# xinge008/SCDA

Measured on AMD Instinct MI355X. Metric: images/sec (fwd+bwd) VGG16 Faster-RCNN+SCDA 512x1024, higher is better.
Workload: dtype f32; 1 GPU; vgg16_FasterRCNN + 4-cluster SCDA, synthetic Cityscapes->Foggy 512x1024, batch=1/GPU (BASELINE.json configs[1]); 1 step = 1 source + 1 target image, 4 optimiser phases; gt_boxes=12, rois=512, clusters=4, recon=256, parallelism=dp1

## Files before the change

include/scda_ops.h:

```cpp
#ifndef SCDA_OPS_H
#define SCDA_OPS_H

#include <stddef.h>
#include <stdint.h>

#ifdef __cplusplus
extern "C" {
#endif

#define SCDA_OK 0
#define SCDA_EINVAL (-1)
#define SCDA_ELAUNCH (-2)
#define SCDA_ENODEV (-3)

int scda_version(void);
int scda_device_count(void);
const char *scda_last_error(void);

void scda_prof_enable(unsigned kernel_mask);
int scda_prof_num_kernels(void);
const char *scda_prof_kernel_name(int k);
int scda_prof_collect(long long *launches, double *ms, double *flops, double *bytes);
void scda_debug_last_plan(int *out4);
void scda_debug_plan_conv(int dir, int batch, int Cin, int IH, int IW, int Cout, int KH, int KW, int S, int P, int row_period,
// ... 46 lines not shown
int scda_bbox_overlaps_hip(const float *boxes, int N, const float *query, int K, float *out, void *stream);

int scda_anchor_label_hip(const float *anchors, int KA, const float *gts, int G, int gt_stride, float neg_thresh, float pos_thresh,
                          float min_gt_best, float *best_iou, int *best_gt, unsigned *gt_best, signed char *labels, int *pos_list,
                          int *neg_list, int *counts, void *stream);
int scda_anchor_finalize_hip(signed char *labels, const int *best_gt, const int *pos_list, const int *drop_pos, int n_drop_pos,
                             const int *neg_list, const int *drop_neg, int n_drop_neg, const double *anchors64, const float *gts,
                             int gt_stride, int A, int fh, int fw, long long *cls_targets, float *loc_targets, float *loc_masks,
                             void *stream);
int scda_proposal_decode_hip(const int *order, const float *exp_wh, int n, const double *anchors64, const float *loc, const float *prob, int A, int fh,
                             int fw, double img_h, double img_w, double min_size, float *props5, unsigned char *ok, void *stream);
int scda_proposal_gather_hip(const float *props5, const long long *keep, const long long *num_keep, float image_index, int max_rows,
                             float *out6, void *stream);
int scda_proposal_match_hip(const float *props, int n_prop, int prop_stride, const float *gts, int G, int gt_stride, float img_h,
                            float img_w, float pos_thresh, float neg_hi, float neg_lo, float *rois, float *best_iou, int *best_gt,
                            signed char *labels, int *pos_list, int *neg_list, int *counts, void *stream);
int scda_proposal_finalize_hip(const float *cand_rois, const int *sel, const int *gt_of, const float *enc, const float *gts,
                               int gt_stride, int R, int num_classes, float image_index, float *rois5, long long *labels,
                               float *loc_targets, float *loc_weights, void *stream);

int scda_kmeans_capacity(void);
int scda_kmeans_hip(const float *rois, int roi_stride, int N, int k, int first_index, const double *uniforms_host, int trials,
                    float *centres, int *labels, int *counts, int *members, int *seed_index, int *n_iter, int *status, void *stream);
int scda_cluster_gather_hip(const float *feats, long long feat_stride, int N, int F, const int *members, const int *counts,
                            const int *picks_or_null, int k, int threshold, float *out, void *stream);

size_t scda_rpn_topk_workspace_bytes(int B, int KA, int top_n);
int scda_rpn_topk_hip(const float *prob, int B, int A, int fh, int fw, int top_n, int *order, void *ws, void *stream);
int scda_rpn_decode_batched_hip(const int *order, int n, const double *anchors64, const float *loc, const float *prob, int B, int A,
                                int fh, int fw, const float *image_info, int info_stride, double min_size, float *props5,
                                unsigned char *ok, void *stream);
size_t scda_rpn_proposals_workspace_bytes(int B, int A, int fh, int fw, int top_n);
int scda_rpn_proposals_hip(const float *prob, const float *loc, const double *anchors64, int B, int A, int fh, int fw,
                           const float *image_info, int info_stride, int pre_nms_top_n, double min_size, float nms_thresh,
                           int post_nms_top_n, void *ws, float *rois5, float *props6, int *counts, void *stream);
size_t scda_box_predict_workspace_bytes(int B, int P, int C);
int scda_box_predict_hip(const float *rois, const int *roi_counts, int B, int P, const float *prob, const float *loc, int C,
                         const float *image_info, int info_stride, const double *stds_host, const double *means_host,
                         float score_thresh, float nms_thresh, int top_n, void *ws, float *det, int *det_counts, void *stream);
int scda_soft_nms_capacity(void);
int scda_soft_nms_segments_hip(float *boxes, const long long *seg, int S, int max_n, int method, float sigma, float Nt, float threshold,
                               int64_t *keep, int64_t *num_out, void *stream);
int scda_box_predict_soft_hip(const float *rois, const int *roi_counts, int B, int P, const float *prob, const float *loc, int C,
                              const float *image_info, int info_stride, const double *stds_host, const double *means_host,
                              float score_thresh, int top_n, int method, float sigma, float Nt, float threshold, void *ws, float *det,
                              int *det_counts, void *stream);

int scda_det_rois_hip(const float *detections, const int *detection_counts, int B, int top_n, float *rois5, int *cls, void *stream);
int scda_mask_select_hip(const float *logits, long long stride_r, long long stride_c, long long stride_h, long long stride_w,
                         const int *cls, int R, int C, int ph, int pw, int sigmoid, float *out, void *stream);
int scda_mask_paste_hip(const float *rois, int roi_stride, const int *cls_or_null, const float *planes, int R, int ph, int pw, int H,
                        int W, int packed, float threshold, void *out, void *stream);
int scda_mask_rescale_max_ratio(void);
int scda_mask_rescale_hip(const float *rois, int roi_stride, const int *cls_or_null, const float *planes, int R, int ph, int pw, int H,
                          int W, const float *image_info, int info_stride, int masks_per_image, int Ho, int Wo, int packed,
                          float threshold, void *out, float *foot_rois, int *status, void *stream);

size_t scda_keypoint_decode_workspace_bytes(int R, int Kp, int W);
int scda_keypoint_decode_hip(const float *rois, int roi_stride, const int *cls_or_null, const float *heat, long long stride_r,
                             long long stride_k, long long stride_h, long long stride_w, int R, int Kp, int ph, int pw, int H, int W,
                             void *workspace, float *out, void *stream);

int scda_keypoint_ce_fwd_hip(const float *heat, long long stride_r, long long stride_k, int R, int Kp, int HW, const int *targets,
                             float *stats, float *row_loss, float *out2, void *stream);
int scda_keypoint_ce_bwd_hip(const float *heat, long long stride_r, long long stride_k, int R, int Kp, int HW, const int *targets,
                             const float *stats, const float *out2, const float *grad_scalar, float *dheat, long long dstride_r,
                             long long dstride_k, void *stream);

int scda_mask_rle_max_chars(int h, int w);
size_t scda_mask_rle_workspace_bytes(int R, int H, int Wd, int cap_runs);
int scda_mask_rle_hip(const uint32_t *bits, int R, int H, int Wd, const float *image_info, int info_stride, int masks_per_image,
                      int h_all, int w_all, const float *rois_or_null, int roi_stride, int cap_runs, int cap_bytes, void *ws,
                      int *n_runs, uint32_t *counts, int *n_bytes, unsigned char *chars, uint32_t *area, uint32_t *bbox, void *stream);
size_t scda_mask_iou_workspace_bytes(int M, int N, int H, int Wd);
int scda_mask_iou_hip(const uint32_t *dt_bits, int M, const uint32_t *gt_bits, int N, int H, int Wd, int h, int w,
                      const unsigned char *iscrowd_or_null, void *ws, double *iou, uint32_t *inter, void *stream);

size_t scda_mask_frpoly_workspace_bytes(int P, int Q, int H, int Wd);
int scda_mask_frpoly_hip(const double *xy, int V, const int *poly_first, const int *poly_plane, int P, const uint32_t *rle_counts, int C,
                         const int *rle_first, const int *rle_plane, int Q, const int *sizes, int N, int H, int Wd, void *ws,
                         uint32_t *bits, uint32_t *area_or_null, void *stream);

int scda_coco_det_rows_hip(const float *detections, const int *detection_counts, int B, int top_n, const uint32_t *mask_area_or_null,
                           int K, double *dt_xywh, double *dt_area, float *score, int *cat, void *stream);
int scda_coco_box_iou_hip(const double *dt, const int *dt_counts, const double *gt, const int *gt_counts, const unsigned char *iscrowd,
                          int B, int D, int G, double *iou, void *stream);
int scda_coco_match_hip(const double *iou, int B, int D, int G, const int *dt_counts, const int *dt_cat, const float *score,
                        const double *dt_area, const int *gt_counts, const int *gt_cat, const double *gt_area,
                        const unsigned char *gt_iscrowd, int K, const double *iou_thrs, int T, const double *area_rng, int A, int max_det,
                        int *rank, uint32_t *bits, int *npig, int *seen, int *dbg_match_or_null, void *stream);
int scda_coco_match_ign_hip(const double *iou, int B, int D, int G, const int *dt_counts, const int *dt_cat, const float *score,
                            const double *dt_area, const int *gt_counts, const int *gt_cat, const double *gt_area,
                            const unsigned char *gt_iscrowd, const unsigned char *gt_ignore_or_null, int K, const double *iou_thrs, int T,
                            const double *area_rng, int A, int max_det, int *rank, uint32_t *bits, int *npig, int *seen,
                            int *dbg_match_or_null, void *stream);
int scda_coco_kp_rows_hip(const float *detections, const int *detection_counts, int B, int top_n, const float *keypoints, int Kp, int K,
                          double *dt_xywh, double *dt_area, float *score, int *cat, void *stream);
int scda_coco_oks_hip(const float *dt_keypoints, const int *dt_counts, const double *gt_keypoints, const double *gt_boxes,
                      const double *gt_areas, const int *gt_counts, const double *vars, int Kp, const unsigned char *gt_iscrowd_or_null,
                      const int *gt_num_keypoints_or_null, int B, int D, int G, double *oks, unsigned char *gt_ignore_or_null,
                      void *stream);
int scda_coco_prop_rows_hip(const float *proposals, const int *proposal_counts, int B, int P, int xyxy_as_xywh, double *dt_xywh,
                            double *dt_area, float *score, int *cat, void *stream);
int scda_coco_regroup_hip(int B, int D, int G, int K, const int *dt_counts, const double *in_xywh, const double *in_area,
                          const float *in_score, const int *in_cat, const int *gt_counts, const int *gt_cat, const double *gt_area,
                          const unsigned char *gt_iscrowd, const double *in_iou, double *dt_xywh, double *dt_area, float *score, int *cat,
                          double *out_gt_area, unsigned char *out_gt_iscrowd, int *out_gt_cat, double *out_iou, int *perm_dets,
                          int *perm_gts, void *stream);
size_t scda_coco_accumulate_workspace_bytes(int n_images, int D, int K, int A);
int scda_coco_accumulate_hip(const int *image_ids, int n_images, int D, const int *cat, const int *rank, const float *score,
                             const uint32_t *bits, const int *npig, const int *seen, int K, int T, int A, const double *rec_thrs, int R,
                             const int *max_dets, int M, int max_det_last, void *ws, double *precision, double *recall, double *scores,
                             void *stream);
int scda_coco_summarize_hip(const double *precision, const double *recall, int T, int R, int K, int A, int M, const int *spec,
                            int n_stats, double *stats, void *stream);

int scda_map_rows_hip(const float *detections, const int *detection_counts, int B, int D, const float *image_info, int info_w,
                      int scale_column, int num_classes, int keep_num, int *box, float *score, int *cls, int *rank, int *kept, int *tp,
                      int *dbg_match_or_null, int G, int *dbg_claimed_or_null, void *stream);
int scda_map_match_hip(const int *box, const int *cls, const int *rank, const int *kept, int B, int D, const int *gt_boxes,
                       const int *gt_counts, int G, int num_classes, double iou_thr, int *tp, int *gt_num, int *dbg_match_or_null,
                       int *dbg_claimed_or_null, void *stream);
int scda_map_recall_hip(const float *proposals, const int *proposal_counts, int B, int P, int prop_w, const float *gts,
                        const int *gt_counts, int Gr, int gt_w, int *counters, void *stream);
size_t scda_map_accumulate_workspace_bytes(int n_images, int D);
int scda_map_accumulate_hip(int n_images, int D, const float *score, const int *cls, const int *rank, const int *kept, const int *tp,
                            const int *sum_gt, int num_classes, void *ws, double *ap, double *max_recall, int *rows, void *stream);

int scda_eval_place_rows_hip(const void *src, int W, int cap, int row_words, const int *order_host, const int *counts_host_or_null,
                             const int *counts_dev_or_null, int start, int max_images, int fill, void *dst, int *flags, void *stream);
int scda_eval_sum_counters_hip(const int *src, int W, int n, int *dst, void *stream);
size_t scda_eval_mark_duplicates_workspace_bytes(int n);
int scda_eval_mark_duplicates_hip(const int *image_ids, int n, void *ws, int *first, int *flags, int raise_on_duplicate, void *stream);
int scda_map_merge_duplicates_hip(const int *first, int n, int D, const int *box, const float *score, const int *cls, const int *rank,
                                  const int *kept, int *tp, int *flags, void *stream);

size_t scda_conv2d_workspace_bytes(int batch, int Cin, int IH, int IW, int Cout, int KH, int KW, int S, int P);
size_t scda_conv2d_packed_elems(int Cout, int Cin, int KH, int KW, int for_dgrad);
int scda_conv2d_pack_weight_hip(const float *w, float *out, int Cout, int Cin, int KH, int KW, int for_dgrad,
                                void *stream);
long long scda_conv2d_pack_tiles(int Cout, int Cin, int KH, int KW, int for_dgrad);
int scda_conv2d_pack_weights_batched_hip(const float *base, float *out, const long long *desc, int n, long long n_tiles,
                                         void *stream);
int scda_conv2d_fwd_hip(const float *x, const float *wp, const float *bias , float *y, int batch,
                        int Cin, int IH, int IW, int Cout, int KH, int KW, int S, int P, int row_period, int act, float slope,
                        void *ws, size_t ws_bytes, void *stream);
int scda_conv2d_dgrad_hip(const float *dy, const float *wt, float *dx, int batch, int Cin, int IH, int IW, int Cout,
                          int KH, int KW, int S, int P, int row_period, void *ws, size_t ws_bytes, void *stream);
int scda_conv2d_dgrad_act_hip(const float *dy, const float *wt, float *dx, int batch, int Cin, int IH, int IW, int Cout,
                              int KH, int KW, int S, int P, int row_period, const float *act_src, float act_slope, void *ws,
                              size_t ws_bytes, void *stream);
int scda_conv2d_dgrad_small_cin_hip(const float *dy, const float *w, float *dx, int batch, int Cin, int IH, int IW, int Cout,
                                    int KH, int KW, int S, int P, void *stream);
int scda_conv2d_wgrad_hip(const float *dy, const float *x, float *dw, int batch, int Cin, int IH, int IW, int Cout,
                          int KH, int KW, int S, int P, int row_period, int accumulate, void *ws, size_t ws_bytes, void *stream);
int scda_conv2d_wgrad_bias_fusable(int batch, int Cout, int OH, int OW, const float *dy);
int scda_conv2d_wgrad_bias_hip(const float *dy, const float *x, float *dw, float *db, int batch, int Cin, int IH, int IW,
                               int Cout, int KH, int KW, int S, int P, int row_period, int accumulate, int db_accumulate, void *ws,
                               size_t ws_bytes, void *stream);

int scda_conv2d_wino_supported(int batch, int C, int H, int W, int M);
size_t scda_conv2d_wino_packed_elems(int Cout, int Cin, int for_dgrad);
int scda_conv2d_wino_pack_hip(const float *w, float *out, int Cout, int Cin, int for_dgrad, void *stream);
int scda_conv2d_wino_hip(const float *x, const float *u, const float *bias, float *y, int batch, int C, int H, int W, int M, int act,
                         float slope, const float *mask_src, float mask_slope, int for_dgrad, void *ws, size_t ws_bytes, void *stream);

int scda_conv2d_wino_stacked_hip(const float *x, const float *u, const float *bias, float *y, int maps, int C, int M, int act, float slope,
                                 const float *mask_src, float mask_slope, int for_dgrad, void *ws, size_t ws_bytes, void *stream);
int scda_conv2d_wino_pool_hip(const float *x, const float *u, const float *bias, float *pool_y, unsigned char *pool_idx, int batch, int C,
                              int H, int W, int M, int act, float slope, void *stream);
int scda_conv2d_wino_wgrad_supported(int batch, int Cin, int H, int W, int Cout);
int scda_conv2d_wino_wgrad_hip(const float *dy, const float *x, float *dw, float *db, int batch, int Cin, int H, int W, int Cout,
                               int accumulate, int db_accumulate, void *ws, size_t ws_bytes, void *stream);
int scda_conv2d_wino_wgrad_stacked_hip(const float *dy, const float *x, float *dw, float *db, int maps, int Cin, int Cout, int accumulate,
                                       int db_accumulate, void *ws, size_t ws_bytes, void *stream);

size_t scda_gemm_workspace_bytes(int M, int N, int K);
int scda_gemm_hip(const float *A, const float *B, float *C, int M, int N, int K, int lda, int ldb, int ldc,
                  int trans_a, int trans_b, const float *bias, int bias_on_n, int act, float slope, int accumulate,
                  void *ws, size_t ws_bytes, void *stream);

int scda_maxpool2x2_fwd_hip(const float *x, float *y, uint8_t *idx, int planes, int H, int W, void *stream);
int scda_maxpool2x2_bwd_hip(const float *dy, const uint8_t *idx, float *dx, int planes, int H, int W, void *stream);
int scda_maxpool3x3s2_fwd_hip(const float *x, float *y, int planes, int H, int W, void *stream);
int scda_add_relu_hip(const float *a, const float *b, float *y, long long n, void *stream);
int scda_maxpool2x2_bwd_relu_hip(const float *dy, const uint8_t *idx, const float *y_pooled, float *dx, int planes, int H, int W,
                                 void *stream);
int scda_act_fwd_hip(const float *x, float *y, long long n, int mode, float slope, void *stream);
int scda_act_bwd_hip(const float *dy, const float *y, float *dx, long long n, int mode, float slope, void *stream);
int scda_axpby_hip(const float *a, const float *b, float *y, long long n, float alpha, float beta, void *stream);
int scda_dropout_mask_hip(uint8_t *mask, long long n, float p, uint64_t seed, void *stream);
int scda_dropout_apply_hip(const float *x, const uint8_t *mask, float *y, long long n, float scale, void *stream);
int scda_dropout_seeded_hip(const float *x, float *y, long long n, float p, uint64_t seed, float scale, const float *relu_src,
                            void *stream);
int scda_sigmoid_bce_rows_fwd_hip(const float *x, const float *t, int t_rows, const float *w, int C, int n, float scale,
                                  int accumulate, float *prob_out, float *out1, void *stream);
int scda_sigmoid_bce_rows_bwd_hip(const float *prob, const float *t, int t_rows, const float *w, int C, int n, float scale,
                                  const float *grad_scalar, float *dx, void *stream);
size_t scda_bias_grad_workspace_bytes(int C);
int scda_bias_grad_nchw_hip(const float *dy, float *db, int B, int C, int HW, int accumulate, float *ws, void *stream);
int scda_colsum_hip(const float *dy, float *db, int M, int N, int accumulate, void *stream);
int scda_softmax_ce_fwd_hip(const float *logits, const int64_t *targets, int R, int C, int ignore_index, float *probs,
                            float *out2, void *stream);
int scda_softmax_ce_bwd_hip(const float *probs, const int64_t *targets, int R, int C, int ignore_index,
                            const float *fwd_out2, const float *grad_scalar, float *dlogits, void *stream);
int scda_row_softmax_hip(const float *x, float *y, int R, int C, void *stream);
int scda_accuracy_hip(const float *logits, const int64_t *targets, int R, int C, int ignore_index, float *out1,
                      void *stream);
size_t scda_smooth_l1_workspace_bytes(void);
int scda_smooth_l1_fwd_hip(const float *pred, const float *mask, const float *target, long long n, float sigma,
                           float scale, float *partial_ws, float *out1, void *stream);
int scda_smooth_l1_bwd_hip(const float *pred, const float *mask, const float *target, long long n, float sigma,
                           float scale, const float *grad_scalar, float *dpred, void *stream);
int scda_instnorm_fwd_hip(const float *x, float *y, float *mean, float *rstd, int planes, int HW, float eps, int act,
                          float slope, void *stream);
int scda_instnorm_bwd_hip(const float *dy, const float *x, const float *mean, const float *rstd, float *dx, int planes,
                          int HW, int act, float slope, void *stream);
int scda_instnorm_drop_add_fwd_hip(const float *x, const float *residual, float *y, float *mean, float *rstd, int planes, int HW,
                                   float eps, float p, uint64_t seed, float scale , void *stream);
int scda_instnorm_drop_bwd_hip(const float *dy, const float *x, const float *mean, const float *rstd, float *dx, int planes, int HW,
                               float p, uint64_t seed, float scale, void *stream);
int scda_instnorm_drop_add_fwd_dev_hip(const float *x, const float *residual, float *y, float *mean, float *rstd, int planes, int HW,
                                       float eps, float p, const uint64_t *seed_dev, float scale, void *stream);
int scda_instnorm_drop_bwd_dev_hip(const float *dy, const float *x, const float *mean, const float *rstd, float *dx, int planes, int HW,
                                   float p, const uint64_t *seed_dev, float scale, void *stream);
size_t scda_batchnorm_workspace_bytes(int B, int C, int HW);
int scda_batchnorm_fwd_hip(const float *x, float *y, const float *gamma, const float *beta, float *running_mean,
                           float *running_var, float *save_mean, float *save_rstd, int B, int C, int HW, float eps,
                           float momentum, int act, float slope, float *ws, void *stream);
int scda_batchnorm_bwd_hip(const float *dy, const float *x, const float *gamma, const float *beta, const float *save_mean,
                           const float *save_rstd, float *dx, float *dgamma, float *dbeta, int B, int C, int HW, int act,
                           float slope, int accumulate, float *ws, void *stream);
int scda_batchnorm_add_relu_ok(int B, int HW);
int scda_batchnorm_add_relu_fwd_hip(const float *x, const float *residual, float *y, const float *gamma, const float *beta,
                                    float *running_mean, float *running_var, float *save_mean, float *save_rstd, int B, int C,
                                    int HW, float eps, float momentum, void *stream);
int scda_batchnorm_add_relu_bwd_hip(const float *dy, const float *x, const float *y, const float *gamma, const float *beta,
                                    const float *save_mean, const float *save_rstd, float *dx_or_null, float *d_residual,
                                    float *dgamma, float *dbeta, int B, int C, int HW, int accumulate, void *stream);
int scda_batchnorm_eval_hip(const float *x, const float *dy_or_null, float *out, const float *gamma, const float *beta,
                            const float *running_mean, const float *running_var, int B, int C, int HW, float eps, int act,
                            float slope, void *stream);
int scda_upsample2x_fwd_hip(const float *x, float *y, int planes, int IH, int IW, void *stream);
int scda_upsample2x_bwd_hip(const float *dy, float *dx, int planes, int IH, int IW, void *stream);
int scda_instnorm_up2_supported(int IH, int IW);
int scda_instnorm_up2_fwd_hip(const float *x, float *y2, float *mean, float *rstd, int planes, int IH, int IW, float eps, int act,
                              float slope, void *stream);
int scda_instnorm_drop_add_up2_fwd_hip(const float *x, const float *residual, float *y2, float *mean, float *rstd, int planes, int IH,
                                       int IW, float eps, float p, uint64_t seed, float scale , void *stream);
int scda_instnorm_drop_add_up2_fwd_dev_hip(const float *x, const float *residual, float *y2, float *mean, float *rstd, int planes,
                                           int IH, int IW, float eps, float p, const uint64_t *seed_dev, float scale, void *stream);
int scda_instnorm_up2_bwd_hip(const float *dy2, const float *x, const float *mean, const float *rstd, float *dx, int planes, int IH,
                              int IW, int act, float slope, void *stream);
int scda_instnorm_drop_up2_bwd_hip(const float *dy2, const float *x, const float *mean, const float *rstd, float *dx, float *dresidual,
                                   int planes, int IH, int IW, float p, uint64_t seed, float scale, void *stream);
int scda_instnorm_drop_up2_bwd_dev_hip(const float *dy2, const float *x, const float *mean, const float *rstd, float *dx,
                                       float *dresidual, int planes, int IH, int IW, float p, const uint64_t *seed_dev, float scale,
                                       void *stream);
int scda_bce_fwd_hip(const float *p, const float *t, int n, float *out1, void *stream);
int scda_bce_bwd_hip(const float *p, const float *t, int n, const float *grad_scalar, float *dp, void *stream);
int scda_avg2x2s1_fwd_hip(const float *x, float *y, int planes, int H, int W, void *stream);
int scda_avg2x2s1_bwd_hip(const float *dy, float *dx, int planes, int H, int W, void *stream);
int scda_gap_fwd_hip(const float *x, float *y, int planes, int HW, void *stream);
int scda_gap_bwd_hip(const float *dy, float *dx, int planes, int HW, void *stream);
int scda_row_mean_hip(const float *x, float *y, int R, int C, void *stream);
int scda_adam_hip(float *param, const float *grad, float *exp_avg, float *exp_avg_sq, long long n, float lr,
                  float beta1, float beta2, float eps, float weight_decay, int step, void *stream);
int scda_adam_limited_hip(float *param, const float *grad, float *exp_avg, float *exp_avg_sq, long long n, float lr,
                          float beta1, float beta2, float eps, float weight_decay, int step, int max_blocks, void *stream);

size_t scda_image_resize_tmp_bytes(int rows, int out_w, int C);
int scda_image_resize_normalize_hip(const unsigned char *src, int H, int W, int C, const int *bounds_h, const int *kk_h,
                                    int ksize_h, int out_w, const int *bounds_v, const int *kk_v, int ksize_v, int out_h,
                                    int row0, int rows, unsigned char *tmp, size_t tmp_bytes, int normalize, float mean,
                                    float stdv, int flip, float *out, void *stream);

#ifdef __cplusplus
}
#endif
#endif
```

scda_amd/native.py:

```python
import ctypes
import os
import re
import weakref

import torch

_HERE = os.path.dirname(os.path.abspath(__file__))
LIB_PATH = os.environ.get("SCDA_OPS_LIB") or os.path.join(_HERE, "libscda_ops.so")
HEADER_PATH = os.path.join(os.path.dirname(_HERE), "include", "scda_ops.h")

_lib = None


class ScdaNativeError(RuntimeError):
    pass


C_SCALARS = {"int": ctypes.c_int, "unsigned": ctypes.c_uint, "float": ctypes.c_float, "double": ctypes.c_double,
             "long long": ctypes.c_longlong, "size_t": ctypes.c_size_t, "uint64_t": ctypes.c_uint64}
C_RETURNS = dict(C_SCALARS, **{"void": None, "const char *": ctypes.c_char_p})


def parse_header(text):
    text = re.sub(r"/\*.*?\*/", " ", text, flags=re.S)
# ... 1088 lines not shown
    return bool(lib().scda_conv2d_wino_enabled())


def _route(direction, B, Cin, IH, IW, Cout, KH, KW, stride, pad, row_period):
    pool, maps = ctypes.c_int(0), ctypes.c_int(0)
    fam = lib().scda_conv2d_route(direction, B, Cin, IH, IW, Cout, KH, KW, stride, pad, row_period, ctypes.byref(pool), ctypes.byref(maps))
    return fam, bool(pool.value), maps.value


def wino_stacked(B, IH, IW, row_period):
    return _route(0, B, 0, IH, IW, 0, 3, 3, 1, 1, row_period)[2]


def wino_ok(B, Cin, IH, IW, Cout, KH, KW, stride, pad, row_period=0):
    return _route(0, B, Cin, IH, IW, Cout, KH, KW, stride, pad, row_period)[0] != 0


def wino_wgrad_ok(B, Cin, IH, IW, Cout, KH, KW, stride, pad, row_period=0):
    return _route(2, B, Cin, IH, IW, Cout, KH, KW, stride, pad, row_period)[0] != 0


def conv2d_wino_wgrad(dy, x, w_shape, out=None, db_out=None, want_bias=False, row_period=0):
    _req(dy, "dy"); _req(x, "x")
    B, Cin, IH, IW = x.shape
    Cout = w_shape[0]
    acc = dbacc = 0
    if out is None:
        out = torch.empty(tuple(w_shape), dtype=torch.float32, device=x.device)
    else:
        _req(out, "out"); acc = 1
    db = None
    if want_bias or db_out is not None:
        if db_out is None:
            db = torch.empty(Cout, dtype=torch.float32, device=x.device)
        else:
            _req(db_out, "db_out"); db = db_out; dbacc = 1
    ws, n = _conv_ws(B, Cin, IH, IW, Cout, 3, 3, 1, 1, x.device)
    if row_period:
        maps = wino_stacked(B, IH, IW, row_period)
        if not maps:
            raise ValueError("conv2d_wino_wgrad: row_period %d on %s is not a stack of 7 x 7 maps" % (row_period, tuple(x.shape)))
        _check(lib().scda_conv2d_wino_wgrad_stacked_hip(_p(dy), _p(x), _p(out), _p(db), maps, Cin, Cout, acc, dbacc, _p(ws), n, _stream()),
               "scda_conv2d_wino_wgrad_stacked_hip")
        return out, db
    _check(lib().scda_conv2d_wino_wgrad_hip(_p(dy), _p(x), _p(out), _p(db), B, Cin, IH, IW, Cout, acc, dbacc, _p(ws), n, _stream()),
           "scda_conv2d_wino_wgrad_hip")
    return out, db


def conv2d_wino_pack(w, for_dgrad=False, cache=True):
    _req(w, "w")
    Cout, Cin, KH, KW = w.shape
    cache = cache and isinstance(w, torch.nn.Parameter)
    key = (w.data_ptr(), 2 + int(for_dgrad))
    flat = getattr(w, "_scda_flat", None)
    tag = (w._version, flat.epoch if flat is not None else WEIGHT_EPOCH[0], tuple(w.shape))
    if cache:
        hit = _PACK_CACHE.get(key)
        if hit is not None and hit[0] == tag and hit[2]() is w:
            return hit[1]
    L = lib()
    n = L.scda_conv2d_wino_packed_elems(Cout, Cin, int(for_dgrad))
    out = torch.empty(n, dtype=torch.float32, device=w.device)
    _check(L.scda_conv2d_wino_pack_hip(_p(w.contiguous()), _p(out), Cout, Cin, int(for_dgrad), _stream()), "scda_conv2d_wino_pack_hip")
    if cache:
        _PACK_CACHE[key] = (tag, out, weakref.ref(w))
    return out


def conv2d_wino(x, u, bias, M, act=ACT_NONE, slope=0.01, mask_src=None, mask_slope=0.0, for_dgrad=False, row_period=0):
    B, C, H, W = x.shape
    y = torch.empty(B, M, H, W, dtype=torch.float32, device=x.device)
    ws, n = _conv_ws(B, C, H, W, M, 3, 3, 1, 1, x.device)
    if row_period:
        maps = wino_stacked(B, H, W, row_period)
        if not maps:
            raise ValueError("conv2d_wino: row_period %d on %s is not a stack of 7 x 7 maps" % (row_period, tuple(x.shape)))
        _check(lib().scda_conv2d_wino_stacked_hip(_p(x), _p(u), _p(bias), _p(y), maps, C, M, act, slope, _p(mask_src), mask_slope,
                                                  int(for_dgrad), _p(ws), n, _stream()), "scda_conv2d_wino_stacked_hip")
        return y
    _check(lib().scda_conv2d_wino_hip(_p(x), _p(u), _p(bias), _p(y), B, C, H, W, M, act, slope, _p(mask_src), mask_slope, int(for_dgrad),
                                      _p(ws), n, _stream()), "scda_conv2d_wino_hip")
    return y


def conv_pool_fusable(B, Cin, IH, IW, Cout, KH, KW, stride, pad, row_period=0):
    return _route(0, B, Cin, IH, IW, Cout, KH, KW, stride, pad, row_period)[1]


def conv2d_wino_pool(x, u, bias, M, act=ACT_NONE, slope=0.01):
    B, C, H, W = x.shape
    y = torch.empty(B, M, H // 2, W // 2, dtype=torch.float32, device=x.device)
    idx = torch.empty(B, M, H // 2, W // 2, dtype=torch.uint8, device=x.device)
    _check(lib().scda_conv2d_wino_pool_hip(_p(x), _p(u), _p(bias), _p(y), _p(idx), B, C, H, W, M, act, slope, _stream()),
           "scda_conv2d_wino_pool_hip")
    return y, idx


def conv2d_pack_all(flat):
    ws = getattr(flat, "conv_weights", None)
    if not ws:
        return
    wino = tuple(bool(getattr(w, "_scda_wino_used", False)) for w in ws) if wino_enabled() else None
    plans = flat.__dict__.setdefault("_scda_pack_plans", {})
    plan = plans.get(wino)
    L = lib()
    if plan is None:
        rows, entries, off, tiles = [], [], 0, 0
        base = flat.data.data_ptr()
        for i, w in enumerate(ws):
            Cout, Cin, KH, KW = w.shape
            src = (w.data_ptr() - base) // 4
            use_wino = wino is not None and wino[i] and all(L.scda_conv2d_packed_elems(Cout, Cin, KH, KW, d) for d in (2, 3))
            for d in ((2, 3) if use_wino else (0, 1)):
                n = int(L.scda_conv2d_packed_elems(Cout, Cin, KH, KW, d))
                rows.append([src, off, Cout, Cin, KH * KW, d, tiles])
                entries.append((w, d if d >= 2 else bool(d), off, n))
                off += n
                tiles += int(L.scda_conv2d_pack_tiles(Cout, Cin, KH, KW, d))
        desc = upload(torch.tensor(rows, dtype=torch.int64), flat.data.device)
        while len(plans) >= 4:
            plans.pop(next(iter(plans)))
        plan = (desc, off, entries, tiles, wino)
    else:
        plans.pop(wino)
    plans[wino] = plan
    desc, total, entries, tiles, _ = plan
    out = flat.__dict__.get("_scda_pack_out")
    if out is None or out.numel() < total:
        out = flat.__dict__["_scda_pack_out"] = torch.empty(total, dtype=torch.float32, device=flat.data.device)
    _check(L.scda_conv2d_pack_weights_batched_hip(_p(flat.data), _p(out), _p(desc), len(entries), tiles, _stream()),
           "scda_conv2d_pack_weights_batched_hip")
    for w, d, off, n in entries:
        if w.data_ptr() < flat.data.data_ptr():
            continue
        _PACK_CACHE[(w.data_ptr(), d)] = ((w._version, flat.epoch, tuple(w.shape)), out[off:off + n], weakref.ref(w))


def conv2d_fwd(x, w, bias, stride, pad, act=ACT_NONE, slope=0.01, row_period=0):
    _req(x, "x"); _req(w, "w")
    if bias is not None:
        _req(bias, "bias")
    B, Cin, IH, IW = x.shape
    Cout, Cin2, KH, KW = w.shape
    if Cin2 != Cin:
        raise ValueError(f"conv2d: input has {Cin} channels, weight expects {Cin2}")
    OH = (IH + 2 * pad - KH) // stride + 1
    OW = (IW + 2 * pad - KW) // stride + 1
    use_wino = wino_ok(B, Cin, IH, IW, Cout, KH, KW, stride, pad, row_period)
    if isinstance(w, torch.nn.Parameter):
        w._scda_wino_used = use_wino
    if use_wino:
        return conv2d_wino(x, conv2d_wino_pack(w, False), bias, Cout, act, slope, row_period=row_period)
    wp = conv2d_pack_weight(w, False)
    y = torch.empty(B, Cout, OH, OW, dtype=torch.float32, device=x.device)
    ws, n = _conv_ws(B, Cin, IH, IW, Cout, KH, KW, stride, pad, x.device)
    _check(lib().scda_conv2d_fwd_hip(_p(x), _p(wp), _p(bias), _p(y), B, Cin, IH, IW, Cout, KH, KW, stride, pad, row_period, act, slope,
                                     _p(ws), n, _stream()), "scda_conv2d_fwd_hip")
    return y


def conv2d_dgrad(dy, w, x_shape, stride, pad, act_src=None, act_slope=0.0, row_period=0):
    _req(dy, "dy"); _req(w, "w")
    B, Cin, IH, IW = x_shape
    Cout, _, KH, KW = w.shape
    if act_src is not None:
        _req(act_src, "act_src")
        if tuple(act_src.shape) != tuple(x_shape):
            raise ValueError("act_src must have the shape of the conv input")
    if _route(1, B, Cin, IH, IW, Cout, KH, KW, stride, pad, row_period)[0]:
        return conv2d_wino(dy, conv2d_wino_pack(w, True), None, Cin, ACT_NONE, 0.0, act_src, act_slope, for_dgrad=True, row_period=row_period)
    dx = torch.empty(B, Cin, IH, IW, dtype=torch.float32, device=dy.device)
    if act_src is None and Cin <= 4 and Cout * KH * KW * 16 <= 65536 and (KH, KW) in ((3, 3), (1, 1)):
        _check(lib().scda_conv2d_dgrad_small_cin_hip(_p(dy), _p(w.contiguous()), _p(dx), B, Cin, IH, IW, Cout, KH, KW, stride, pad,
                                                     _stream()), "scda_conv2d_dgrad_small_cin_hip")
        return dx
    wt = conv2d_pack_weight(w, True)
    ws, n = _conv_ws(B, Cin, IH, IW, Cout, KH, KW, stride, pad, dy.device)
    _check(lib().scda_conv2d_dgrad_act_hip(_p(dy), _p(wt), _p(dx), B, Cin, IH, IW, Cout, KH, KW, stride, pad, row_period, _p(act_src),
                                           act_slope, _p(ws), n, _stream()), "scda_conv2d_dgrad_act_hip")
    return dx


def conv2d_wgrad(dy, x, w_shape, stride, pad, out=None, row_period=0):
    _req(dy, "dy"); _req(x, "x")
    B, Cin, IH, IW = x.shape
    Cout, _, KH, KW = w_shape
    if wino_wgrad_ok(B, Cin, IH, IW, Cout, KH, KW, stride, pad, row_period):
        return conv2d_wino_wgrad(dy, x, w_shape, out=out, row_period=row_period)[0]
    acc = 0
    if out is None:
        out = torch.empty(tuple(w_shape), dtype=torch.float32, device=x.device)
    else:
        _req(out, "out"); acc = 1
    ws, n = _conv_ws(B, Cin, IH, IW, Cout, KH, KW, stride, pad, x.device)
    _check(lib().scda_conv2d_wgrad_hip(_p(dy), _p(x), _p(out), B, Cin, IH, IW, Cout, KH, KW, stride, pad, row_period, acc, _p(ws), n,
                                       _stream()), "scda_conv2d_wgrad_hip")
    return out


def conv2d_wgrad_bias(dy, x, w_shape, stride, pad, out=None, db_out=None, row_period=0):
    _req(dy, "dy"); _req(x, "x")
    B, Cin, IH, IW = x.shape
    Cout, _, KH, KW = w_shape
    if wino_wgrad_ok(B, Cin, IH, IW, Cout, KH, KW, stride, pad, row_period):
        return conv2d_wino_wgrad(dy, x, w_shape, out=out, db_out=db_out, want_bias=True, row_period=row_period)
    L = lib()
    if not L.scda_conv2d_wgrad_bias_fusable(B, Cout, dy.shape[2], dy.shape[3], _p(dy)):
        return conv2d_wgrad(dy, x, w_shape, stride, pad, out=out, row_period=row_period), bias_grad_nchw(dy, out=db_out)
    acc = dbacc = 0
    if out is None:
        out = torch.empty(tuple(w_shape), dtype=torch.float32, device=x.device)
    else:
        _req(out, "out"); acc = 1
    if db_out is None:
        db_out = torch.empty(Cout, dtype=torch.float32, device=x.device)
    else:
        _req(db_out, "db_out"); dbacc = 1
    ws, n = _conv_ws(B, Cin, IH, IW, Cout, KH, KW, stride, pad, x.device)
    _check(L.scda_conv2d_wgrad_bias_hip(_p(dy), _p(x), _p(out), _p(db_out), B, Cin, IH, IW, Cout, KH, KW, stride, pad, row_period, acc,
                                        dbacc, _p(ws), n, _stream()), "scda_conv2d_wgrad_bias_hip")
    return out, db_out


def gemm(a, b, M, N, K, lda, ldb, trans_a=False, trans_b=False, bias=None, bias_on_n=True, act=ACT_NONE, slope=0.01,
         out=None, accumulate=False):
    _req(a, "a"); _req(b, "b")
    if out is None:
        if accumulate:
            raise ValueError("accumulate needs out")
        out = torch.empty(M, N, dtype=torch.float32, device=a.device)
    else:
        _req(out, "out")
    L = lib()
    n = L.scda_gemm_workspace_bytes(M, N, K)
    ws = workspace(n, a.device)
    _check(L.scda_gemm_hip(_p(a), _p(b), _p(out), M, N, K, lda, ldb, N, int(trans_a), int(trans_b), _p(bias), int(bias_on_n), act, slope,
                           int(accumulate), _p(ws), n, _stream()), "scda_gemm_hip")
    return out


def linear_fwd(x, w, bias, act=ACT_NONE):
    M, K = x.shape
    N = w.shape[0]
    return gemm(x, w, M, N, K, K, K, False, False, bias, True, act)


def linear_dgrad(dy, w):
    M, K = dy.shape
    N = w.shape[1]
    return gemm(dy, w, M, N, K, K, N, False, True)


def linear_wgrad(dy, x, out=None, accumulate=True):
    Kb, M = dy.shape
    N = x.shape[1]
    return gemm(dy, x, M, N, Kb, M, N, True, True, out=out, accumulate=out is not None and accumulate)


def maxpool2x2_fwd(x):
    _req(x, "x")
    B, C, H, W = x.shape
    y = torch.empty(B, C, H // 2, W // 2, dtype=torch.float32, device=x.device)
    idx = torch.empty(B, C, H // 2, W // 2, dtype=torch.uint8, device=x.device)
    _check(lib().scda_maxpool2x2_fwd_hip(_p(x), _p(y), _p(idx), B * C, H, W, _stream()), "scda_maxpool2x2_fwd_hip")
    return y, idx


def maxpool2x2_bwd(dy, idx, x_shape, relu_y=None):
    _req(dy, "dy"); _req(idx, "idx", torch.uint8)
    B, C, H, W = x_shape
    dx = torch.empty(B, C, H, W, dtype=torch.float32, device=dy.device)
    if relu_y is None:
        _check(lib().scda_maxpool2x2_bwd_hip(_p(dy), _p(idx), _p(dx), B * C, H, W, _stream()), "scda_maxpool2x2_bwd_hip")
    else:
        _req(relu_y, "relu_y")
        _check(lib().scda_maxpool2x2_bwd_relu_hip(_p(dy), _p(idx), _p(relu_y), _p(dx), B * C, H, W, _stream()),
               "scda_maxpool2x2_bwd_relu_hip")
    return dx


def maxpool3x3s2_fwd(x):
    _req(x, "x")
    B, C, H, W = x.shape
    y = torch.empty(B, C, (H - 1) // 2 + 1, (W - 1) // 2 + 1, dtype=torch.float32, device=x.device)
    _check(lib().scda_maxpool3x3s2_fwd_hip(_p(x), _p(y), B * C, H, W, _stream()), "scda_maxpool3x3s2_fwd_hip")
    return y


def add_relu(a, b):
    _req(a, "a"); _req(b, "b")
    if a.shape != b.shape:
        raise ValueError("add_relu: shape mismatch")
    y = torch.empty_like(a)
    _check(lib().scda_add_relu_hip(_p(a), _p(b), _p(y), a.numel(), _stream()), "scda_add_relu_hip")
    return y


ACT_MODE = {"relu": 0, "leaky": 1, "tanh": 2, "sigmoid": 3}


def act_fwd(x, mode, slope=0.01):
    _req(x, "x")
    y = torch.empty_like(x)
    _check(lib().scda_act_fwd_hip(_p(x), _p(y), x.numel(), mode, slope, _stream()), "scda_act_fwd_hip")
    return y


def act_bwd(dy, y, mode, slope=0.01):
    _req(dy, "dy"); _req(y, "y")
    dx = torch.empty_like(dy)
    _check(lib().scda_act_bwd_hip(_p(dy), _p(y), _p(dx), dy.numel(), mode, slope, _stream()), "scda_act_bwd_hip")
    return dx


def axpby(a, b, alpha=1.0, beta=1.0):
    _req(a, "a")
    if b is not None:
        _req(b, "b")
    y = torch.empty_like(a)
    _check(lib().scda_axpby_hip(_p(a), _p(b), _p(y), a.numel(), alpha, beta, _stream()), "scda_axpby_hip")
    return y


def dropout_mask(shape, p, seed, device):
    mask = torch.empty(shape, dtype=torch.uint8, device=device)
    _check(lib().scda_dropout_mask_hip(_p(mask), mask.numel(), p, seed & 0xFFFFFFFFFFFFFFFF, _stream()), "scda_dropout_mask_hip")
    return mask


def dropout_apply(x, mask, scale):
    _req(x, "x"); _req(mask, "mask", torch.uint8)
    y = torch.empty_like(x)
    _check(lib().scda_dropout_apply_hip(_p(x), _p(mask), _p(y), x.numel(), scale, _stream()), "scda_dropout_apply_hip")
    return y


def dropout_seeded(x, p, seed, scale, relu_src=None):
    _req(x, "x")
    if relu_src is not None:
        _req(relu_src, "relu_src")
    y = torch.empty_like(x)
    _check(lib().scda_dropout_seeded_hip(_p(x), _p(y), x.numel(), p, seed & 0xFFFFFFFFFFFFFFFF, scale, _p(relu_src), _stream()),
           "scda_dropout_seeded_hip")
    return y


def sigmoid_bce_rows_fwd(x, t, w, scale, out=None, want_prob=True):
    _req(x, "x"); _req(t, "t")
    C, n = x.shape
    t_rows = t.numel() // n
    if t.numel() != t_rows * n or t_rows not in (1, C):
        raise ValueError("labels must be [1,n] or [C,n]")
    if w is not None:
        _req(w, "w")
    acc = out is not None
    if out is None:
        out = torch.empty(1, dtype=torch.float32, device=x.device)
    prob = torch.empty_like(x) if want_prob else None
# ... 454 lines not shown
```

Before: 113.2 images/s.

## Add dedicated thin-channel 1x1 conv kernels for fwd, dgrad and wgrad

```diff
diff --git a/include/scda_ops.h b/include/scda_ops.h
--- a/include/scda_ops.h
+++ b/include/scda_ops.h
@@ -222,6 +222,14 @@
                               size_t ws_bytes, void *stream);
 int scda_conv2d_dgrad_small_cin_hip(const float *dy, const float *w, float *dx, int batch, int Cin, int IH, int IW, int Cout,
                                     int KH, int KW, int S, int P, void *stream);
+int scda_conv1x1_thin_ok(int batch, int Cin, int IH, int IW, int Cout, int KH, int KW, int S, int P, int row_period);
+int scda_conv1x1_thin_fwd_hip(const float *x, const float *w, const float *bias , float *y, int batch, int Cin, int HW,
+                              int Cout, int act, float slope, void *stream);
+int scda_conv1x1_thin_dgrad_hip(const float *dy, const float *w, float *dx, int batch, int Cin, int HW, int Cout, const float *act_src,
+                                float act_slope, void *stream);
+size_t scda_conv1x1_thin_wgrad_workspace_bytes(int batch, int Cin, int HW, int Cout);
+int scda_conv1x1_thin_wgrad_hip(const float *dy, const float *x, float *dw, float *db, int batch, int Cin, int HW, int Cout,
+                                int accumulate, int db_accumulate, void *ws, size_t ws_bytes, void *stream);
 int scda_conv2d_wgrad_hip(const float *dy, const float *x, float *dw, int batch, int Cin, int IH, int IW, int Cout,
                           int KH, int KW, int S, int P, int row_period, int accumulate, void *ws, size_t ws_bytes, void *stream);
 int scda_conv2d_wgrad_bias_fusable(int batch, int Cout, int OH, int OW, const float *dy);
diff --git a/scda_amd/csrc/conv_thin.hip b/scda_amd/csrc/conv_thin.hip
--- /dev/null
+++ b/scda_amd/csrc/conv_thin.hip
@@ -0,0 +1,332 @@
+#include <hip/hip_runtime.h>
+#include <stdint.h>
+
+#include <algorithm>
+
+#include "common.h"
+#include "launch_plan.h"
+#include "mfma_tile.h"
+
+namespace scda {
+
+constexpr int THIN_MAX = 4;
+constexpr int THIN_LDS_ROWS = 1024;
+constexpr long long THIN_MIN_PIXELS = 65536;
+constexpr int THIN_WG_FC = 8;
+constexpr int THIN_WG_STRIP = 1024;
+
+template <int PX> struct PxVec;
+template <> struct PxVec<4> {
+    static __device__ __forceinline__ void load(const float *p, float v[4]) { const float4 t = *reinterpret_cast<const float4 *>(p); v[0] = t.x; v[1] = t.y; v[2] = t.z; v[3] = t.w; }
+    static __device__ __forceinline__ void store(float *p, const float v[4]) { *reinterpret_cast<float4 *>(p) = make_float4(v[0], v[1], v[2], v[3]); }
+};
+template <> struct PxVec<1> {
+    static __device__ __forceinline__ void load(const float *p, float v[1]) { v[0] = *p; }
+    static __device__ __forceinline__ void store(float *p, const float v[1]) { *p = v[0]; }
+};
+
+__device__ __forceinline__ void thin_stage_weights(const float *__restrict__ w, double *wl, const int rows, const int cols, const int srow,
+                                                   const int scol) {
+    for (int i = threadIdx.x; i < rows * THIN_MAX; i += blockDim.x) {
+        const int r = i >> 2, c = i & 3;
+        wl[i] = c < cols ? (double)w[(size_t)r * srow + (size_t)c * scol] : 0.0;
+    }
+    __syncthreads();
+}
+
+template <int M, int PX>
+__global__ __launch_bounds__(256) void conv1x1_thin_rows_kernel(const float *__restrict__ in, const float *__restrict__ w, const int sm,
+                                                                const int sk, const float *__restrict__ bias, float *__restrict__ out,
+                                                                const long long groups, const int K, const int HW, const int act,
+                                                                const float slope, const float *__restrict__ mask_src,
+                                                                const float mask_slope) {
+    extern __shared__ __attribute__((aligned(16))) double thin_wl[];
+    double *part = thin_wl + (size_t)K * THIN_MAX;
+    thin_stage_weights(w, thin_wl, K, M, sk, sm);
+    const int lane = threadIdx.x & 63, wave = __builtin_amdgcn_readfirstlane(threadIdx.x >> 6);
+    const int kq = (K + 3) >> 2, k0 = wave * kq, k1 = min(K, k0 + kq);
+    const int gpi = HW / PX;
+    const long long tiles = (groups + 63) >> 6;
+    for (long long tile = blockIdx.x; tile < tiles; tile += gridDim.x) {
+        const long long gidx = tile * 64 + lane;
+        const bool live = gidx < groups;
+        const long long b = live ? gidx / gpi : 0;
+        const int p = live ? (int)(gidx - b * gpi) * PX : 0;
+        const float *src = in + (size_t)b * K * HW + p;
+        double acc[M][PX];
+#pragma unroll
+        for (int m = 0; m < M; ++m)
+#pragma unroll
+            for (int j = 0; j < PX; ++j) acc[m][j] = 0.0;
+        if (live) {
+#pragma unroll 8
+            for (int k = k0; k < k1; ++k) {
+                float v[PX];
+                PxVec<PX>::load(src + (size_t)k * HW, v);
+#pragma unroll
+                for (int m = 0; m < M; ++m) {
+                    const double a = thin_wl[k * THIN_MAX + m];
+#pragma unroll
+                    for (int j = 0; j < PX; ++j) acc[m][j] = fma(a, (double)v[j], acc[m][j]);
+                }
+            }
+        }
+        if (wave > 0) {
+#pragma unroll
+            for (int m = 0; m < M; ++m)
+#pragma unroll
+                for (int j = 0; j < PX; ++j) part[((wave - 1) * (M * PX) + m * PX + j) * 64 + lane] = acc[m][j];
+        }
+        __syncthreads();
+        if (wave == 0 && live) {
+#pragma unroll
+            for (int m = 0; m < M; ++m) {
+                const size_t o = ((size_t)b * M + m) * HW + p;
+                float r[PX], ms[PX];
+                if (mask_src) PxVec<PX>::load(mask_src + o, ms);
+#pragma unroll
+                for (int j = 0; j < PX; ++j) {
+                    double t = acc[m][j];
+#pragma unroll
+                    for (int q = 0; q < 3; ++q) t += part[(q * (M * PX) + m * PX + j) * 64 + lane];
+                    float x = (float)(bias ? t + (double)bias[m] : t);
+                    x = apply_act(x, act, slope);
+                    if (mask_src) x = ms[j] > 0.f ? x : x * mask_slope;
+                    r[j] = x;
+                }
+                PxVec<PX>::store(out + o, r);
+            }
+        }
+        __syncthreads();
+    }
+}
+
+template <int K, int PX>
+__global__ __launch_bounds__(256) void conv1x1_thin_k_kernel(const float *__restrict__ in, const float *__restrict__ w, const int sm,
+                                                             const int sk, const float *__restrict__ bias, float *__restrict__ out,
+                                                             const long long groups, const int M, const int mper, const int HW,
+                                                             const int act, const float slope, const float *__restrict__ mask_src,
+                                                             const float mask_slope) {
+    extern __shared__ __attribute__((aligned(16))) double thin_wl[];
+    const int m0 = blockIdx.y * mper, m1 = min(M, m0 + mper);
+    thin_stage_weights(w + (size_t)m0 * sm, thin_wl, m1 - m0, K, sm, sk);
+    const int gpi = HW / PX;
+    for (long long gidx = blockIdx.x * 256LL + threadIdx.x; gidx < groups; gidx += gridDim.x * 256LL) {
+        const long long b = gidx / gpi;
+        const int p = (int)(gidx - b * gpi) * PX;
+        double v[K][PX];
+#pragma unroll
+        for (int k = 0; k < K; ++k) {
+            float t[PX];
+            PxVec<PX>::load(in + ((size_t)b * K + k) * HW + p, t);
+#pragma unroll
+            for (int j = 0; j < PX; ++j) v[k][j] = (double)t[j];
+        }
+#pragma unroll 4
+        for (int m = m0; m < m1; ++m) {
+            const size_t o = ((size_t)b * M + m) * HW + p;
+            float r[PX], ms[PX];
+            if (mask_src) PxVec<PX>::load(mask_src + o, ms);
+            const double bm = bias ? (double)bias[m] : 0.0;
+#pragma unroll
+            for (int j = 0; j < PX; ++j) {
+                double a = 0.0;
+#pragma unroll
+                for (int k = 0; k < K; ++k) a = fma(thin_wl[(m - m0) * THIN_MAX + k], v[k][j], a);
+                float x = (float)(bias ? a + bm : a);
+                x = apply_act(x, act, slope);
+                if (mask_src) x = ms[j] > 0.f ? x : x * mask_slope;
+                r[j] = x;
+            }
+            PxVec<PX>::store(out + o, r);
+        }
+    }
+}
+
+template <int TC, int PX>
+__global__ __launch_bounds__(256) void conv1x1_thin_wgrad_kernel(const float *__restrict__ T, const float *__restrict__ F, const int FC_all,
+                                                                 const long long npix, const int HW, double *__restrict__ part) {
+    constexpr int FC = THIN_WG_FC, NV = TC * FC + TC + FC;
+    __shared__ double red[4][NV];
+    const int f0 = blockIdx.y * FC, nf = min(FC, FC_all - f0);
+    const long long n0 = (long long)blockIdx.x * THIN_WG_STRIP, n1 = min(npix, n0 + THIN_WG_STRIP);
+    double acc[NV];
+#pragma unroll
+    for (int i = 0; i < NV; ++i) acc[i] = 0.0;
+    for (long long n = n0 + (long long)threadIdx.x * PX; n < n1; n += 256 * PX) {
+        const long long b = n / HW;
+        const int p = (int)(n - b * HW);
+        double tv[TC][PX];
+#pragma unroll
+        for (int t = 0; t < TC; ++t) {
+            float v[PX];
+            PxVec<PX>::load(T + ((size_t)b * TC + t) * HW + p, v);
+#pragma unroll
+            for (int j = 0; j < PX; ++j) { tv[t][j] = (double)v[j]; acc[TC * FC + t] += tv[t][j]; }
+        }
+#pragma unroll
+        for (int f = 0; f < FC; ++f) {
+            if (f < nf) {
+                float v[PX];
+                PxVec<PX>::load(F + ((size_t)b * FC_all + f0 + f) * HW + p, v);
+#pragma unroll
+                for (int j = 0; j < PX; ++j) {
+                    const double fv = (double)v[j];
+                    acc[TC * FC + TC + f] += fv;
+#pragma unroll
+                    for (int t = 0; t < TC; ++t) acc[t * FC + f] = fma(tv[t][j], fv, acc[t * FC + f]);
+                }
+            }
+        }
+    }
+    const int lane = threadIdx.x & 63, wave = threadIdx.x >> 6;
+#pragma unroll
+    for (int i = 0; i < NV; ++i) {
+        double v = acc[i];
+#pragma unroll
+        for (int off = 32; off > 0; off >>= 1) v += __shfl_xor(v, off, 64);
+        if (lane == 0) red[wave][i] = v;
+    }
+    __syncthreads();
+    if (threadIdx.x < NV) {
+        const int i = threadIdx.x;
+        const double s = ((red[0][i] + red[1][i]) + red[2][i]) + red[3][i];
+        const int E = TC * FC_all + TC + FC_all;
+        double *row = part + (size_t)blockIdx.x * E;
+        if (i < TC * FC) {
+            const int t = i / FC, f = i - t * FC;
+            if (f < nf) row[t * FC_all + f0 + f] = s;
+        } else if (i < TC * FC + TC) {
+            if (blockIdx.y == 0) row[TC * FC_all + (i - TC * FC)] = s;
+        } else {
+            const int f = i - TC * FC - TC;
+            if (f < nf) row[TC * FC_all + TC + f0 + f] = s;
+        }
+    }
+}
+
+__global__ __launch_bounds__(256) void conv1x1_thin_wgrad_reduce_kernel(const double *__restrict__ part, const int strips, const int TC,
+                                                                        const int FC_all, const int thin_is_cout, float *__restrict__ dw,
+                                                                        const int accumulate, float *__restrict__ db,
+                                                                        const int db_accumulate) {
+    const int E = TC * FC_all + TC + FC_all;
+    const int lane = threadIdx.x & 63;
+    const int e = blockIdx.x * 4 + (threadIdx.x >> 6);
+    if (e >= E) return;
+    double s = 0.0;
+    for (int i = lane; i < strips; i += 64) s += part[(size_t)i * E + e];
+#pragma unroll
+    for (int off = 32; off > 0; off >>= 1) s += __shfl_xor(s, off, 64);
+    if (lane != 0) return;
+    if (e < TC * FC_all) {
+        const int t = e / FC_all, f = e - t * FC_all;
+        float *dst = dw + (thin_is_cout ? t * FC_all + f : f * TC + t);
+        *dst = (float)(accumulate ? s + (double)*dst : s);
+        return;
+    }
+    const int q = e - TC * FC_all;
+    const bool of_t = q < TC;
+    if (!db || of_t != (thin_is_cout != 0)) return;
+    float *dst = db + (of_t ? q : q - TC);
+    *dst = (float)(db_accumulate ? s + (double)*dst : s);
+}
+
+static bool thin_aligned16(const void *a, const void *b = nullptr, const void *c = nullptr) {
+    return ((((uintptr_t)a) | ((uintptr_t)b) | ((uintptr_t)c)) & 15) == 0;
+}
+
+static int thin_apply(const char *who, const float *in, const float *w, int sm, int sk, const float *bias, float *out, int batch, int K, int M,
+                      int HW, int act, float slope, const float *mask_src, float mask_slope, hipStream_t st) {
+    const bool vec = (HW & 3) == 0 && thin_aligned16(in, out, mask_src);
+    const int px = vec ? 4 : 1;
+    const long long groups = (long long)batch * (HW / px);
+    const unsigned gx = (unsigned)std::min<long long>((groups + 255) / 256, 1 << 20);
+    if (M <= THIN_MAX) {
+        if (K > THIN_LDS_ROWS) { set_error("%s: %d channels do not fit the weights' LDS image", who, K); return SCDA_EINVAL; }
+        const unsigned gt = (unsigned)std::min<long long>((groups + 63) / 64, 1 << 20);
+#define THIN_ROWS(M_)                                                                                                                      \
+        do {                                                                                                                                   \
+            if (vec) hipLaunchKernelGGL((conv1x1_thin_rows_kernel<M_, 4>), dim3(gt), dim3(256), ((size_t)K * THIN_MAX + 3 * M_ * 4 * 64) * sizeof(double), st, in, w, sm, sk, bias, out, groups, K, HW, act, slope, mask_src, mask_slope); \
+            else hipLaunchKernelGGL((conv1x1_thin_rows_kernel<M_, 1>), dim3(gt), dim3(256), ((size_t)K * THIN_MAX + 3 * M_ * 64) * sizeof(double), st, in, w, sm, sk, bias, out, groups, K, HW, act, slope, mask_src, mask_slope);    \
+        } while (0)
+        if (M == 1) THIN_ROWS(1); else if (M == 2) THIN_ROWS(2); else if (M == 3) THIN_ROWS(3); else THIN_ROWS(4);
+#undef THIN_ROWS
+        return launch_status("conv1x1_thin_rows_kernel");
+    }
+    if (K > THIN_MAX) { set_error("%s: neither side has at most %d channels", who, THIN_MAX); return SCDA_EINVAL; }
+    const int mper = 16, gy = (M + mper - 1) / mper;
+    if (gy > 65535) { set_error("%s: %d output channels are too many", who, M); return SCDA_EINVAL; }
+    const size_t lds = (size_t)mper * THIN_MAX * sizeof(double);
+#define THIN_K(K_)                                                                                                                         \
+    do {                                                                                                                                   \
+        if (vec) hipLaunchKernelGGL((conv1x1_thin_k_kernel<K_, 4>), dim3(gx, gy), dim3(256), lds, st, in, w, sm, sk, bias, out, groups, M, mper, HW, act, slope, mask_src, mask_slope); \
+        else hipLaunchKernelGGL((conv1x1_thin_k_kernel<K_, 1>), dim3(gx, gy), dim3(256), lds, st, in, w, sm, sk, bias, out, groups, M, mper, HW, act, slope, mask_src, mask_slope);    \
+    } while (0)
+    if (K == 1) THIN_K(1); else if (K == 2) THIN_K(2); else if (K == 3) THIN_K(3); else THIN_K(4);
+#undef THIN_K
+    return launch_status("conv1x1_thin_k_kernel");
+}
+
+SCDA_API int scda_conv1x1_thin_ok(int batch, int Cin, int IH, int IW, int Cout, int KH, int KW, int S, int P, int row_period) {
+    if (batch <= 0 || Cin <= 0 || Cout <= 0 || IH <= 0 || IW <= 0 || KH != 1 || KW != 1 || S != 1 || P != 0 || row_period != 0) return 0;
+    if (std::min(Cin, Cout) > THIN_MAX || std::max(Cin, Cout) > THIN_LDS_ROWS) return 0;
+    if ((long long)IH * IW > 0x7fffffffLL || (long long)batch * IH * IW < THIN_MIN_PIXELS) return 0;
+    return lp::read_plan_env().force.set ? 0 : 1;
+}
+
+SCDA_API int scda_conv1x1_thin_fwd_hip(const float *x, const float *w, const float *bias, float *y, int batch, int Cin, int HW, int Cout,
+                                       int act, float slope, void *stream) {
+    if (!x || !w || !y || batch <= 0 || Cin <= 0 || Cout <= 0 || HW <= 0) { set_error("scda_conv1x1_thin_fwd_hip: bad arguments"); return SCDA_EINVAL; }
+    return thin_apply("scda_conv1x1_thin_fwd_hip", x, w, Cin, 1, bias, y, batch, Cin, Cout, HW, act, slope, nullptr, 0.f, as_stream(stream));
+}
+
+SCDA_API int scda_conv1x1_thin_dgrad_hip(const float *dy, const float *w, float *dx, int batch, int Cin, int HW, int Cout,
+                                         const float *act_src, float act_slope, void *stream) {
+    if (!dy || !w || !dx || batch <= 0 || Cin <= 0 || Cout <= 0 || HW <= 0) { set_error("scda_conv1x1_thin_dgrad_hip: bad arguments"); return SCDA_EINVAL; }
+    return thin_apply("scda_conv1x1_thin_dgrad_hip", dy, w, 1, Cin, nullptr, dx, batch, Cout, Cin, HW, (int)ACT_NONE, 0.f, act_src, act_slope,
+                      as_stream(stream));
+}
+
+SCDA_API size_t scda_conv1x1_thin_wgrad_workspace_bytes(int batch, int Cin, int HW, int Cout) {
+    const long long npix = (long long)batch * HW;
+    const long long strips = (npix + THIN_WG_STRIP - 1) / THIN_WG_STRIP;
+    return (size_t)strips * ((size_t)Cin * Cout + Cin + Cout) * sizeof(double);
+}
+
+SCDA_API int scda_conv1x1_thin_wgrad_hip(const float *dy, const float *x, float *dw, float *db, int batch, int Cin, int HW, int Cout,
+                                         int accumulate, int db_accumulate, void *ws, size_t ws_bytes, void *stream) {
+    if (!dy || !x || !dw || batch <= 0 || Cin <= 0 || Cout <= 0 || HW <= 0 || std::min(Cin, Cout) > THIN_MAX) {
+        set_error("scda_conv1x1_thin_wgrad_hip: bad arguments");
+        return SCDA_EINVAL;
+    }
+    if (!ws || (((uintptr_t)ws) & 7) || ws_bytes < scda_conv1x1_thin_wgrad_workspace_bytes(batch, Cin, HW, Cout)) {
+        set_error("scda_conv1x1_thin_wgrad_hip: workspace of %zu bytes is too small or misaligned", ws_bytes);
+        return SCDA_EINVAL;
+    }
+    const int thin_is_cout = Cout <= Cin;
+    const float *T = thin_is_cout ? dy : x, *F = thin_is_cout ? x : dy;
+    const int TC = thin_is_cout ? Cout : Cin, FC_all = thin_is_cout ? Cin : Cout;
+    const long long npix = (long long)batch * HW;
+    const long long strips = (npix + THIN_WG_STRIP - 1) / THIN_WG_STRIP;
+    const int runs = (FC_all + THIN_WG_FC - 1) / THIN_WG_FC;
+    if (strips > 0x7fffffffLL || runs > 65535) { set_error("scda_conv1x1_thin_wgrad_hip: problem too large"); return SCDA_EINVAL; }
+    const bool vec = (HW & 3) == 0 && thin_aligned16(T, F);
+    hipStream_t st = as_stream(stream);
+    const dim3 grid((unsigned)strips, (unsigned)runs);
+    double *part = (double *)ws;
+#define THIN_WG(TC_)                                                                                                                       \
+    do {                                                                                                                                   \
+        if (vec) hipLaunchKernelGGL((conv1x1_thin_wgrad_kernel<TC_, 4>), grid, dim3(256), 0, st, T, F, FC_all, npix, HW, part);            \
+        else hipLaunchKernelGGL((conv1x1_thin_wgrad_kernel<TC_, 1>), grid, dim3(256), 0, st, T, F, FC_all, npix, HW, part);                \
+    } while (0)
+    if (TC == 1) THIN_WG(1); else if (TC == 2) THIN_WG(2); else if (TC == 3) THIN_WG(3); else THIN_WG(4);
+#undef THIN_WG
+    int rc = launch_status("conv1x1_thin_wgrad_kernel");
+    if (rc) return rc;
+    const int E = TC * FC_all + TC + FC_all;
+    hipLaunchKernelGGL(conv1x1_thin_wgrad_reduce_kernel, dim3((E + 3) / 4), dim3(256), 0, st, (const double *)part, (int)strips, TC, FC_all,
+                       thin_is_cout, dw, accumulate, db, db_accumulate);
+    return launch_status("conv1x1_thin_wgrad_reduce_kernel");
+}
+
+}
diff --git a/scda_amd/native.py b/scda_amd/native.py
--- a/scda_amd/native.py
+++ b/scda_amd/native.py
@@ -1264,12 +1264,64 @@
         w._scda_wino_used = use_wino
     if use_wino:
         return conv2d_wino(x, conv2d_wino_pack(w, False), bias, Cout, act, slope, row_period=row_period)
+    if conv1x1_thin_ok(B, Cin, IH, IW, Cout, KH, KW, stride, pad, row_period):
+        return conv1x1_thin_fwd(x, w, bias, act, slope)
     wp = conv2d_pack_weight(w, False)
     y = torch.empty(B, Cout, OH, OW, dtype=torch.float32, device=x.device)
     ws, n = _conv_ws(B, Cin, IH, IW, Cout, KH, KW, stride, pad, x.device)
     _check(lib().scda_conv2d_fwd_hip(_p(x), _p(wp), _p(bias), _p(y), B, Cin, IH, IW, Cout, KH, KW, stride, pad, row_period, act, slope,
                                      _p(ws), n, _stream()), "scda_conv2d_fwd_hip")
     return y
+
+
+def conv1x1_thin_ok(B, Cin, IH, IW, Cout, KH, KW, stride, pad, row_period=0):
+    return bool(lib().scda_conv1x1_thin_ok(B, Cin, IH, IW, Cout, KH, KW, stride, pad, row_period))
+
+
+def conv1x1_thin_fwd(x, w, bias, act=ACT_NONE, slope=0.01):
+    _req(x, "x"); _req(w, "w")
+    if bias is not None:
+        _req(bias, "bias")
+    B, Cin, IH, IW = x.shape
+    Cout = w.shape[0]
+    y = torch.empty(B, Cout, IH, IW, dtype=torch.float32, device=x.device)
+    _check(lib().scda_conv1x1_thin_fwd_hip(_p(x), _p(w), _p(bias), _p(y), B, Cin, IH * IW, Cout, act, slope, _stream()),
+           "scda_conv1x1_thin_fwd_hip")
+    return y
+
+
+def conv1x1_thin_dgrad(dy, w, x_shape, act_src=None, act_slope=0.0, out=None):
+    _req(dy, "dy"); _req(w, "w")
+    if act_src is not None:
+        _req(act_src, "act_src")
+    B, Cin, IH, IW = x_shape
+    Cout = w.shape[0]
+    dx = out if out is not None else torch.empty(B, Cin, IH, IW, dtype=torch.float32, device=dy.device)
+    _check(lib().scda_conv1x1_thin_dgrad_hip(_p(dy), _p(w), _p(dx), B, Cin, IH * IW, Cout, _p(act_src), act_slope, _stream()),
+           "scda_conv1x1_thin_dgrad_hip")
+    return dx
+
+
+def conv1x1_thin_wgrad(dy, x, w_shape, out=None, db_out=None, want_bias=False):
+    _req(dy, "dy"); _req(x, "x")
+    B, Cin, IH, IW = x.shape
+    Cout = w_shape[0]
+    acc = dbacc = 0
+    if out is None:
+        out = torch.empty(tuple(w_shape), dtype=torch.float32, device=x.device)
+    else:
+        _req(out, "out"); acc = 1
+    db = None
+    if want_bias or db_out is not None:
+        if db_out is None:
+            db = torch.empty(Cout, dtype=torch.float32, device=x.device)
+        else:
+            _req(db_out, "db_out"); db = db_out; dbacc = 1
+    n = lib().scda_conv1x1_thin_wgrad_workspace_bytes(B, Cin, IH * IW, Cout)
+    ws = workspace(n, x.device)
+    _check(lib().scda_conv1x1_thin_wgrad_hip(_p(dy), _p(x), _p(out), _p(db), B, Cin, IH * IW, Cout, acc, dbacc, _p(ws), n, _stream()),
+           "scda_conv1x1_thin_wgrad_hip")
+    return out, db
 
 
 def conv2d_dgrad(dy, w, x_shape, stride, pad, act_src=None, act_slope=0.0, row_period=0):
@@ -1283,6 +1335,8 @@
     if _route(1, B, Cin, IH, IW, Cout, KH, KW, stride, pad, row_period)[0]:
         return conv2d_wino(dy, conv2d_wino_pack(w, True), None, Cin, ACT_NONE, 0.0, act_src, act_slope, for_dgrad=True, row_period=row_period)
     dx = torch.empty(B, Cin, IH, IW, dtype=torch.float32, device=dy.device)
+    if conv1x1_thin_ok(B, Cin, IH, IW, Cout, KH, KW, stride, pad, row_period):
+        return conv1x1_thin_dgrad(dy, w, x_shape, act_src, act_slope, out=dx)
     if act_src is None and Cin <= 4 and Cout * KH * KW * 16 <= 65536 and (KH, KW) in ((3, 3), (1, 1)):
         _check(lib().scda_conv2d_dgrad_small_cin_hip(_p(dy), _p(w.contiguous()), _p(dx), B, Cin, IH, IW, Cout, KH, KW, stride, pad,
                                                      _stream()), "scda_conv2d_dgrad_small_cin_hip")
@@ -1300,6 +1354,8 @@
     Cout, _, KH, KW = w_shape
     if wino_wgrad_ok(B, Cin, IH, IW, Cout, KH, KW, stride, pad, row_period):
         return conv2d_wino_wgrad(dy, x, w_shape, out=out, row_period=row_period)[0]
+    if conv1x1_thin_ok(B, Cin, IH, IW, Cout, KH, KW, stride, pad, row_period):
+        return conv1x1_thin_wgrad(dy, x, w_shape, out=out)[0]
     acc = 0
     if out is None:
         out = torch.empty(tuple(w_shape), dtype=torch.float32, device=x.device)
@@ -1317,6 +1373,8 @@
     Cout, _, KH, KW = w_shape
     if wino_wgrad_ok(B, Cin, IH, IW, Cout, KH, KW, stride, pad, row_period):
         return conv2d_wino_wgrad(dy, x, w_shape, out=out, db_out=db_out, want_bias=True, row_period=row_period)
+    if conv1x1_thin_ok(B, Cin, IH, IW, Cout, KH, KW, stride, pad, row_period):
+        return conv1x1_thin_wgrad(dy, x, w_shape, out=out, db_out=db_out, want_bias=True)
     L = lib()
     if not L.scda_conv2d_wgrad_bias_fusable(B, Cout, dy.shape[2], dy.shape[3], _p(dy)):
         return conv2d_wgrad(dy, x, w_shape, stride, pad, out=out, row_period=row_period), bias_grad_nchw(dy, out=db_out)
```

Measured after the change: 110.6 images/s. 0.977x the previous value.
